# yahoo/CaffeOnSpark

Hardware: AMD Instinct MI355X
Metric: images/sec (higher is better)
Workload: dtype bf16; 1 GPU; model=alexnet(bvlc_reference/CaffeNet), global_batch=256, parallelism=dp1

## Files before the change

caffeonspark_amd/ops/csrc/ext.cpp:

```cpp

#include <torch/extension.h>
#include <ATen/hip/HIPContext.h>

#include <cstdint>

typedef struct ihipStream_t* hipStream_t;

namespace cosamd {

void gemm_bf16(const void* A, const void* B, void* C, const float* bias,
               int M, int N, int K, int lda, int ldb, int ldc,
               bool trans_a, bool trans_b, int store_mode, int splitk,
               bool relu, float alpha, int m_alloc, int n_alloc,
               hipStream_t stream);
void gemm_f32(const float* A, const float* B, float* C, const float* bias,
              int M, int N, int K, int64_t lda, int64_t ldb, int64_t ldc,
              bool trans_a, bool trans_b, int splitk, bool relu,
              hipStream_t stream);
void im2col_f32(const float* x, float* col, int N, int H, int W, int P,
                int Q, int R, int S, int sh, int sw, int ph, int pw, int dh,
                int dw, int c0, int Cg, int64_t sN, int64_t sC, int64_t sH,
                int64_t sW, hipStream_t stream);
void col2im_f32(const float* dcol, float* dx, int N, int H, int W, int P,
                int Q, int R, int S, int sh, int sw, int ph, int pw, int dh,
                int dw, int c0, int Cg, int64_t sN, int64_t sC, int64_t sH,
                int64_t sW, hipStream_t stream);
void gemm_conv_fwd(const void* X, const void* B, void* C,
                   const float* bias, const void* zpage, int M, int N,
                   int K, int ldb, int ldc, bool relu, bool accum,
                   const int* geom, hipStream_t stream);
void gemm_conv_dw(const void* A, const void* X, float* C,
                  const void* zpage, int M, int N, int K, int lda, int ldc,
                  int store_mode, int splitk, float alpha, float* db,
                  const int* geom, hipStream_t stream);
void gemm_conv_fwd_sc(const void* X, const void* B, void* C,
                      const float* bias, int M, int N, int K, int ldb,
                      int ldc, bool relu, const int* geom,
                      hipStream_t stream);
void gemm_conv_dw_sc(const void* A, const void* X, float* C, int M,
                     int N, int K, int lda, int ldc, int store_mode,
                     int splitk, float alpha, float* db, const int* geom,
                     hipStream_t stream);
void repack_weights(const int64_t* table, int ndesc, int64_t max_total,
                    hipStream_t stream);
void dw_unpack_acc(const float* dwp, float* arena, int Kout, int Cg,
                   int R, int S, int Kpad, bool accumulate,
                   hipStream_t stream);
void s2d_pack(const void* x, void* out, int N, int H, int W, int C, int st,
              int ph, int pw, int Hp, int Wp, int64_t sN, int64_t sC,
              int64_t sH, int64_t sW, hipStream_t stream);
void s2d_pack_weight(const void* src, void* dst, int Kout, int Cg, int R,
                     int S, int st, int Kpad, hipStream_t stream);
void d2s_pack_weight(const void* src, void* dst, int Ci, int Co, int R,
// ... 234 lines not shown
                     (int)x.size(0), (int)x.size(2), (int)x.size(3), (int)P,
                     (int)Q, (int)R, (int)S, (int)sh, (int)sw, (int)ph,
                     (int)pw, (int)dh, (int)dw, (int)c0, (int)Cg,
                     x.stride(0), x.stride(1), x.stride(2), x.stride(3),
                     cur_stream());
}

void py_col2im_f32(Tensor dcol, Tensor dx, int64_t P, int64_t Q, int64_t R,
                   int64_t S, int64_t sh, int64_t sw, int64_t ph, int64_t pw,
                   int64_t dh, int64_t dw, int64_t c0, int64_t Cg) {
  check_conv_f32(dx, dcol, P, Q, R, S, sh, sw, ph, pw, dh, dw, c0, Cg);
  cosamd::col2im_f32(dcol.data_ptr<float>(), dx.data_ptr<float>(),
                     (int)dx.size(0), (int)dx.size(2), (int)dx.size(3),
                     (int)P, (int)Q, (int)R, (int)S, (int)sh, (int)sw,
                     (int)ph, (int)pw, (int)dh, (int)dw, (int)c0, (int)Cg,
                     dx.stride(0), dx.stride(1), dx.stride(2), dx.stride(3),
                     cur_stream());
}

void py_gemm_conv_fwd(Tensor X, Tensor B, Tensor C,
                      c10::optional<Tensor> bias, Tensor zpage,
                      int64_t M, int64_t N, int64_t K, int64_t ldb,
                      int64_t ldc, bool relu, bool accum,
                      std::vector<int64_t> geom) {
  CHECK_CUDA(X); CHECK_BF16(X); CHECK_BF16(B); CHECK_BF16(C);
  const float* bptr = nullptr;
  if (bias.has_value()) {
    CHECK_F32(bias.value());
    bptr = bias.value().data_ptr<float>();
  }
  int g[14];
  TORCH_CHECK(geom.size() == 14, "geom must have 14 ints");
  for (int i = 0; i < 14; ++i) g[i] = (int)geom[i];
  cosamd::gemm_conv_fwd(X.data_ptr(), B.data_ptr(), C.data_ptr(), bptr,
                        zpage.data_ptr(), (int)M, (int)N, (int)K,
                        (int)ldb, (int)ldc, relu, accum, g,
                        cur_stream());
}

void py_gemm_conv_dw(Tensor A, Tensor X, Tensor C,
                     c10::optional<Tensor> db, Tensor zpage, int64_t M,
                     int64_t N,
                     int64_t K, int64_t lda, int64_t ldc,
                     int64_t store_mode, int64_t splitk, double alpha,
                     std::vector<int64_t> geom) {
  CHECK_CUDA(A); CHECK_BF16(A); CHECK_BF16(X); CHECK_F32(C);
  CHECK_CUDA(zpage); CHECK_BF16(zpage);
  TORCH_CHECK(zpage.numel() >= 8, "zpage must hold 16 zero bytes");
  float* dbp = nullptr;
  if (db.has_value()) {
    CHECK_F32(db.value());
    dbp = db.value().data_ptr<float>();
  }
  int g[14];
  TORCH_CHECK(geom.size() == 14, "geom must have 14 ints");
  for (int i = 0; i < 14; ++i) g[i] = (int)geom[i];
  cosamd::gemm_conv_dw(A.data_ptr(), X.data_ptr(), C.data_ptr<float>(),
                       zpage.data_ptr(), (int)M, (int)N, (int)K, (int)lda, (int)ldc,
                       (int)store_mode, (int)splitk, (float)alpha, dbp,
                       g, cur_stream());
// ... 548 lines not shown
  cosamd::softmax_loss_fwd(x.data_ptr(), label.data_ptr<float>(),
                           prob.data_ptr<float>(),
                           rowloss.data_ptr<float>(), loss.data_ptr<float>(),
                           count.data_ptr<int>(), x.size(0), x.size(1),
                           (int)ignore, has_ignore, cur_stream());
}

void py_softmax_loss_bwd(Tensor prob, Tensor label, Tensor dx, double scale,
                         int64_t ignore, bool has_ignore) {
  cosamd::softmax_loss_bwd(prob.data_ptr<float>(), label.data_ptr<float>(),
                           dx.data_ptr(), scale, prob.size(0), prob.size(1),
                           (int)ignore, has_ignore, cur_stream());
}

}

PYBIND11_MODULE(TORCH_EXTENSION_NAME, m) {
  m.def("gemm", &py_gemm);
  m.def("gemm_f32", &py_gemm_f32);
  m.def("im2col_f32", &py_im2col_f32);
  m.def("col2im_f32", &py_col2im_f32);
  m.def("relu_colsum_bwd", &py_relu_colsum_bwd);
  m.def("relu_db_dense", &py_relu_db_dense);
  m.def("gemm_conv_fwd", &py_gemm_conv_fwd);
  m.def("gemm_conv_dw", &py_gemm_conv_dw);
  m.def("gemm_conv_fwd_sc", &py_gemm_conv_fwd_sc);
  m.def("gemm_conv_dw_sc", &py_gemm_conv_dw_sc);
  m.def("im2col", &py_im2col);
  m.def("bn_stats", [](Tensor x, Tensor sum, Tensor sq, int64_t rows,
                       int64_t C) {
    cosamd::bn_stats(x.data_ptr(), sum.data_ptr<float>(),
                     sq.data_ptr<float>(), rows, C, cur_stream());
  });
  m.def("bn_bwd_sums", [](Tensor dy, Tensor xhat, Tensor s1, Tensor s2,
                          int64_t rows, int64_t C) {
    cosamd::bn_bwd_sums(dy.data_ptr(), xhat.data_ptr(),
                        s1.data_ptr<float>(), s2.data_ptr<float>(), rows,
                        C, cur_stream());
  });
  m.def("bn_norm", [](Tensor x, Tensor y, Tensor mean, Tensor invstd,
                      int64_t rows, int64_t C) {
    cosamd::bn_norm(x.data_ptr(), y.data_ptr(), mean.data_ptr<float>(),
                    invstd.data_ptr<float>(), rows, C, cur_stream());
  });
  m.def("bn_bwd", [](Tensor xhat, Tensor dy, Tensor dx, Tensor invstd,
                     Tensor s1, Tensor s2, double inv_m, int64_t rows,
                     int64_t C) {
// ... 75 lines not shown
```

caffeonspark_amd/ops/csrc/gemm.hip:

```cpp

#include "common.h"

#include <type_traits>

namespace cosamd {

typedef __bf16 bf16x8 __attribute__((ext_vector_type(8)));
typedef unsigned short short8v __attribute__((ext_vector_type(8)));
typedef float f32x4 __attribute__((ext_vector_type(4)));

constexpr int BM = 128, BN = 128, BK = 32;
constexpr int NTHREADS = 256;

__device__ __forceinline__ int swz_chunk(int row, int chunk) {
  return chunk ^ ((row >> 1) & 3);
}


struct Tile { int bm, bn, tile_m, tile_n; };

template <int TBN>
__device__ __forceinline__ Tile decode_tile(int M, int N) {
  int mblocks = (M + BM - 1) / BM;
  int nblocks = (N + TBN - 1) / TBN;
  int bid = xcd_swizzle(blockIdx.x, mblocks * nblocks);
  Tile t;
  t.bm = bid / nblocks;
  t.bn = bid % nblocks;
  t.tile_m = t.bm * BM;
  t.tile_n = t.bn * TBN;
  return t;
}

constexpr int mrows_of(int waves) { return BM / (waves / 2); }
constexpr int mfrags_of(int waves) { return mrows_of(waves) / 16; }

template <int MF, int MROWS, bool PRIO>
__device__ __forceinline__ void load_frags_mfma(
    const bf16* As, const bf16* Bs, int wm, int wn, int lane,
    f32x4 (&acc)[MF][4]) {
  int lrow = lane & 15, lchunk = lane >> 4;
  bf16x8 afrag[MF], bfrag[4];
#pragma unroll
  for (int f = 0; f < 4; ++f) {
    int rb = wn * 64 + f * 16 + lrow;
    bfrag[f] = *reinterpret_cast<const bf16x8*>(
        Bs + rb * BK + (swz_chunk(rb, lchunk) << 3));
  }
#pragma unroll
  for (int f = 0; f < MF; ++f) {
    int ra = wm * MROWS + f * 16 + lrow;
    afrag[f] = *reinterpret_cast<const bf16x8*>(
        As + ra * BK + (swz_chunk(ra, lchunk) << 3));
  }
  if (PRIO) __builtin_amdgcn_s_setprio(1);
#pragma unroll
  for (int fm = 0; fm < MF; ++fm)
#pragma unroll
    for (int fn = 0; fn < 4; ++fn)
      acc[fm][fn] = __builtin_amdgcn_mfma_f32_16x16x32_bf16(
          afrag[fm], bfrag[fn], acc[fm][fn], 0, 0, 0);
  if (PRIO) __builtin_amdgcn_s_setprio(0);
}

template <int MF, int MROWS, class Accum>
__device__ __forceinline__ void epilogue_bf16(
    const f32x4 (&acc)[MF][4], bf16* C, const float* bias, int M, int N,
    int ldc, int tile_m, int tile_n, int wm, int wn, int lane, int relu,
    float alpha, Accum accum) {
  int crow0 = tile_m + wm * MROWS + ((lane >> 4) << 2);
  int ccol0 = tile_n + wn * 64 + (lane & 15);
#pragma unroll
  for (int fm = 0; fm < MF; ++fm) {
#pragma unroll
    for (int fn = 0; fn < 4; ++fn) {
      int col = ccol0 + fn * 16;
      if (col >= N) continue;
      float badd = (bias != nullptr) ? bias[col] : 0.f;
#pragma unroll
      for (int r = 0; r < 4; ++r) {
        int row = crow0 + fm * 16 + r;
        if (row >= M) continue;
        float v = acc[fm][fn][r] * alpha + badd;
        if (relu && v < 0.f) v = 0.f;
        int64_t off = (int64_t)row * ldc + col;
        if (accum) v += bf2f(C[off]);
        C[off] = f2bf(v);
      }
    }
  }
}

template <int STORE, bool BIAS, int MF, int MROWS>
__device__ __forceinline__ void epilogue_f32(
    const f32x4 (&acc)[MF][4], float* C, const float* bias, int M, int N,
    int ldc, int tile_m, int tile_n, int wm, int wn, int lane, int relu,
    float alpha) {
  int crow0 = tile_m + wm * MROWS + ((lane >> 4) << 2);
  int ccol0 = tile_n + wn * 64 + (lane & 15);
#pragma unroll
  for (int fm = 0; fm < MF; ++fm) {
#pragma unroll
    for (int fn = 0; fn < 4; ++fn) {
      int col = ccol0 + fn * 16;
      if (col >= N) continue;
      float badd = (BIAS && bias != nullptr) ? bias[col] : 0.f;
#pragma unroll
      for (int r = 0; r < 4; ++r) {
        int row = crow0 + fm * 16 + r;
        if (row >= M) continue;
        float v = acc[fm][fn][r] * alpha;
        if (BIAS) {
// ... 64 lines not shown
    int m0 = (slot >> 4) * 8;
    unsigned short va[8], vb[8];
#pragma unroll
    for (int h = 0; h < 2; ++h) {
      unsigned short* v = h ? vb : va;
      int gk = k0 + kp * 2 + h;
      int gr = row0 + m0;
      if (gk < kend && gr + 8 <= rows && ((ld | gr) % 8 == 0)) {
        *reinterpret_cast<short8v*>(v) =
            *reinterpret_cast<const short8v*>(g + (int64_t)gk * ld + gr);
      } else if (gk < kend) {
#pragma unroll
        for (int j = 0; j < 8; ++j)
          v[j] = (gr + j < rows) ? g[(int64_t)gk * ld + gr + j] : 0;
      } else {
#pragma unroll
        for (int j = 0; j < 8; ++j) v[j] = 0;
      }
    }
    write_kpairs(lds, m0, kp, va, vb);
  }
}

template <int WAVES = 4>
__device__ __forceinline__ void stage_direct_fast(
    bf16* lds, const bf16* g, int row0, int ld, int k0, int tid) {
  int wave = tid >> 6, lane = tid & 63;
  constexpr int CPW = 8 / WAVES;
#pragma unroll
  for (int it = 0; it < CPW; ++it) {
    int chunk = wave * CPW + it;
    int idx = chunk * 512 + lane * 8;
    int row = idx >> 5;
    int kk = swz_chunk(row, (idx & 31) >> 3) << 3;
    auto* gp = (const __attribute__((address_space(1))) unsigned int*)(
        g + (int64_t)(row0 + row) * ld + k0 + kk);
    auto* lp = (__attribute__((address_space(3))) unsigned int*)(
        lds + chunk * 512);
    __builtin_amdgcn_global_load_lds(gp, lp, 16, 0, 0);
  }
}


struct CGeom {
  int H, W, C;
  int Q, PQ;
  int sh, sw, ph, pw, dil, S;
  int c0, Cg;
  int Kcol;
  unsigned long long mPQ, mQ, mCg, mS;
};

__device__ __forceinline__ unsigned mdiv(unsigned n,
                                         unsigned long long m) {
  return (unsigned)(((unsigned long long)n * m) >> 40);
}

static inline unsigned long long magic40(unsigned d) {
  return ((1ull << 40) + d - 1) / d;
}

__device__ __forceinline__ void decode_rows(int* rinfo, const CGeom& gm,
                                            int tile_m, int M, int rows,
                                            int tid) {
  for (int i = tid; i < rows; i += blockDim.x) {
    int m = tile_m + i;
    if (m >= M) m = M - 1;
    unsigned n = mdiv(m, gm.mPQ);
    unsigned pq = m - n * gm.PQ;
    unsigned p = mdiv(pq, gm.mQ);
    unsigned q = pq - p * gm.Q;
    rinfo[i * 3] = (int)(n * gm.H * gm.W);
    rinfo[i * 3 + 1] = (int)p * gm.sh - gm.ph;
    rinfo[i * 3 + 2] = (int)q * gm.sw - gm.pw;
  }
}

template <int WAVES>
__device__ __forceinline__ void stage_implicit_fast(
    bf16* lds_, const bf16* X, const bf16* zpage, const CGeom& gm,
    const int* rinfo, int k0, int tid) {
  auto* lds = reinterpret_cast<unsigned short*>(lds_);
  int wave = tid >> 6, lane = tid & 63;
  constexpr int CPW = 8 / WAVES;
#pragma unroll
  for (int it = 0; it < CPW; ++it) {
    int chunk = wave * CPW + it;
    int idx = chunk * 512 + lane * 8;
    int row = idx >> 5;
    int kk = swz_chunk(row, (idx & 31) >> 3) << 3;
    int k = k0 + kk;
    unsigned rs = mdiv(k, gm.mCg);
    int c = k - rs * gm.Cg;
    unsigned r = mdiv(rs, gm.mS);
    int s = rs - r * gm.S;
    int h = rinfo[row * 3 + 1] + (int)r * gm.dil;
    int w = rinfo[row * 3 + 2] + s * gm.dil;
    bool ok = (k < gm.Kcol) && (h >= 0) && (h < gm.H) && (w >= 0) &&
              (w < gm.W);
    int64_t off = ((int64_t)rinfo[row * 3] +
                   (int64_t)(h * gm.W + w)) * gm.C + gm.c0 + c;
    const bf16* src = ok ? X + off : zpage;
    auto* lp = (__attribute__((address_space(3))) unsigned int*)(
        lds + chunk * 512);
    auto* gp = (const __attribute__((address_space(1))) unsigned int*)src;
    __builtin_amdgcn_global_load_lds(gp, lp, 16, 0, 0);
  }
// ... 220 lines not shown
                             BM);
    bstage.stage(Bs, tile_n, N, k0, k_end, tid);
    __syncthreads();
    if (do_db && tid < BM && tile_m + tid < M) {
      float acc_b = 0.f;
      const bf16* row = As + tid * BK;
#pragma unroll
      for (int kk = 0; kk < BK; ++kk)
        acc_b += bf2f(row[(swz_chunk(tid, kk >> 3) << 3) | (kk & 7)]);
      atomicAdd(db + tile_m + tid, acc_b);
    }
    load_frags_mfma<4, 64, false>(As, Bs, wm, wn, lane, acc);
    __syncthreads();
  }

  epilogue_f32<STORE, false, 4, 64>(acc, C, nullptr, M, N, ldc, tile_m,
                                    tile_n, wm, wn, lane, 0, alpha);
}


struct ADirect {
  const bf16* A;
  int row0, ld;
  template <int WAVES>
  __device__ __forceinline__ void stage(bf16* lds, int k0, int tid) const {
    stage_direct_fast<WAVES>(lds, A, row0, ld, k0, tid);
  }
};

struct AImplicit {
  const bf16* X;
  const bf16* zpage;
  const CGeom& gm;
  const int* rinfo;
  template <int WAVES>
  __device__ __forceinline__ void stage(bf16* lds, int k0, int tid) const {
    stage_implicit_fast<WAVES>(lds, X, zpage, gm, rinfo, k0, tid);
  }
};

template <int N>
__device__ __forceinline__ void wait_vmcnt() {
  asm volatile("s_waitcnt vmcnt(%0)" ::"n"(N) : "memory");
}

template <int WAVES, int DEPTH, class AStage>
__device__ __forceinline__ void pipelined_loop(
    bf16 (*Asb)[BM * BK], bf16 (*Bsb)[BN * BK], const AStage& astage,
    const bf16* B, int tile_n, int ldb, int k_begin, int k_end, int tid,
    int wm, int wn, int lane, f32x4 (&acc)[mfrags_of(WAVES)][4]) {
  constexpr int PF = DEPTH / 2;
  constexpr int VMCNT = PF * 2 * (8 / WAVES);
#pragma unroll
  for (int p = 0; p < PF; ++p)
    if (p == 0 || k_begin + p * BK < k_end) {
      astage.template stage<WAVES>(Asb[p], k_begin + p * BK, tid);
      stage_direct_fast<WAVES>(Bsb[p], B, tile_n, ldb, k_begin + p * BK,
                               tid);
    }
  int cur = 0;
  for (int k0 = k_begin; k0 < k_end; k0 += BK) {
    if (k0 + PF * BK < k_end) {
      int nxt = (cur + PF) & (DEPTH - 1);
      astage.template stage<WAVES>(Asb[nxt], k0 + PF * BK, tid);
      stage_direct_fast<WAVES>(Bsb[nxt], B, tile_n, ldb, k0 + PF * BK,
                               tid);
    }
    wait_vmcnt<VMCNT>();
    __builtin_amdgcn_sched_barrier(0);
    __builtin_amdgcn_s_barrier();
    load_frags_mfma<mfrags_of(WAVES), mrows_of(WAVES), true>(
        Asb[cur], Bsb[cur], wm, wn, lane, acc);
    if (DEPTH == 2) __builtin_amdgcn_s_barrier();
    cur = (cur + 1) & (DEPTH - 1);
  }
}


template <bool TRANS_A, bool TRANS_B, int STORE_MODE, int WAVES = 4>
__global__ __launch_bounds__(WAVES * 64, 2) void gemm_kernel(
    const bf16* __restrict__ A, const bf16* __restrict__ B,
    void* __restrict__ C, const float* __restrict__ bias,
    int M, int N, int K, int lda, int ldb, int ldc,
    int ksplit, int relu, float alpha, int m_alloc, int n_alloc,
    int64_t sA, int64_t sB, int64_t sC) {
  A += (int64_t)blockIdx.z * sA;
  B += (int64_t)blockIdx.z * sB;
  C = (void*)((char*)C + (int64_t)blockIdx.z * sC);
  __shared__ bf16 Asb[2][BM * BK];
  __shared__ bf16 Bsb[2][BN * BK];

  Tile t = decode_tile<BN>(M, N);
  int tile_m = t.tile_m, tile_n = t.tile_n;
  int k_begin = blockIdx.y * ksplit;
  int k_end = min(K, k_begin + ksplit);

  constexpr int NT = WAVES * 64;
  constexpr int MROWS = mrows_of(WAVES), MF = mfrags_of(WAVES);
  int tid = threadIdx.x;
  int wave = tid >> 6, lane = tid & 63;
  int wm = wave >> 1, wn = wave & 1;

  f32x4 acc[MF][4] = {};

  bool a_fast = !TRANS_A && (tile_m + BM <= m_alloc) && (lda % 8 == 0) &&
                ((k_end - k_begin) % BK == 0) && (k_begin % 8 == 0);
  bool b_fast = !TRANS_B && (tile_n + BN <= n_alloc) && (ldb % 8 == 0) &&
                ((k_end - k_begin) % BK == 0) && (k_begin % 8 == 0);

  if (a_fast && b_fast && (k_end - k_begin) >= 2 * BK) {
    pipelined_loop<WAVES, 2>(Asb, Bsb, ADirect{A, tile_m, lda}, B, tile_n,
                             ldb, k_begin, k_end, tid, wm, wn, lane, acc);
  } else {
    bf16* As = Asb[0];
    bf16* Bs = Bsb[0];
    for (int k0 = k_begin; k0 < k_end; k0 += BK) {
      if (a_fast) {
        stage_direct_fast<WAVES>(As, A, tile_m, lda, k0, tid);
      } else if (TRANS_A) {
        stage_trans_pair_guarded(As, A, tile_m, M, lda, k0, k_end, tid,
                                 NT);
      } else {
        stage_direct_guarded(As, A, tile_m, M, lda, k0, k_end, tid, NT);
      }
      if (b_fast) {
        stage_direct_fast<WAVES>(Bs, B, tile_n, ldb, k0, tid);
      } else if (TRANS_B) {
        stage_trans_pair_guarded(Bs, B, tile_n, N, ldb, k0, k_end, tid,
                                 NT);
      } else {
        stage_direct_guarded(Bs, B, tile_n, N, ldb, k0, k_end, tid, NT);
      }
      __syncthreads();
      load_frags_mfma<MF, MROWS, false>(As, Bs, wm, wn, lane, acc);
      __syncthreads();
    }
  }

  if (STORE_MODE == 0 || STORE_MODE == 3)
    epilogue_bf16<MF, MROWS>(acc, reinterpret_cast<bf16*>(C), bias, M, N,
                             ldc, tile_m, tile_n, wm, wn, lane, relu, alpha,
                             std::bool_constant<STORE_MODE == 3>{});
  else
    epilogue_f32<STORE_MODE, true, MF, MROWS>(
        acc, reinterpret_cast<float*>(C), bias, M, N, ldc, tile_m, tile_n,
        wm, wn, lane, relu, alpha);
}


template <int WAVES, int DEPTH>
__global__ __launch_bounds__(WAVES * 64, 2) void gemm_conv_fwd_kernel(
    const bf16* __restrict__ X, const bf16* __restrict__ B,
    bf16* __restrict__ C, const float* __restrict__ bias,
    const bf16* __restrict__ zpage,
    int M, int N, int K, int ldb, int ldc, int relu, int accum,
    CGeom gm) {
  __shared__ bf16 Asb[DEPTH][BM * BK];
  __shared__ bf16 Bsb[DEPTH][BN * BK];
  __shared__ int rinfo[BM * 3];

  Tile t = decode_tile<BN>(M, N);
  int tid = threadIdx.x;
  int wave = tid >> 6, lane = tid & 63;
  int wm = wave >> 1, wn = wave & 1;

  decode_rows(rinfo, gm, t.tile_m, M, BM, tid);
  __syncthreads();

  f32x4 acc[mfrags_of(WAVES)][4] = {};
  pipelined_loop<WAVES, DEPTH>(Asb, Bsb, AImplicit{X, zpage, gm, rinfo}, B,
                               t.tile_n, ldb, 0, K, tid, wm, wn, lane, acc);
  epilogue_bf16<mfrags_of(WAVES), mrows_of(WAVES)>(
      acc, C, bias, M, N, ldc, t.tile_m, t.tile_n, wm, wn, lane, relu, 1.f,
      accum != 0);
}

template <int WAVES>
__global__ __launch_bounds__(WAVES * 64, 2) void gemm_conv_fwd_sc_kernel(
    const bf16* __restrict__ X, const bf16* __restrict__ B,
    bf16* __restrict__ C, const float* __restrict__ bias,
    int M, int N, int K, int ldb, int ldc, int relu, CGeom gm) {
  __shared__ bf16 Asb[2][BM * BK];
  __shared__ bf16 Bsb[2][BN * BK];
  __shared__ int rinfo[BM * 3];

  Tile tl = decode_tile<BN>(M, N);
  constexpr int NT = WAVES * 64;
  constexpr int MROWS = mrows_of(WAVES), MF = mfrags_of(WAVES);
  int tid = threadIdx.x;
  int wave = tid >> 6, lane = tid & 63;
  int wm = wave >> 1, wn = wave & 1;

  decode_rows(rinfo, gm, tl.tile_m, M, BM, tid);
  __syncthreads();

  f32x4 acc[MF][4] = {};
  int T = K / BK;
// ... 266 lines not shown
  }
  else if (!trans_a && trans_b)  COS_GEMM_SM(false, true);
  else if (trans_a && !trans_b)  COS_GEMM_SM(true, false);
  else                           COS_GEMM_SM(true, true);
#undef COS_GEMM_SM
#undef COS_GEMM_CASE
#undef COS_GEMM_CASE8
}

static CGeom make_geom(const int* g) {
  CGeom gm;
  gm.H = g[0]; gm.W = g[1]; gm.C = g[2];
  gm.Q = g[4]; gm.PQ = g[3] * g[4];
  gm.sh = g[5]; gm.sw = g[6]; gm.ph = g[7]; gm.pw = g[8];
  gm.dil = g[9]; gm.S = g[10];
  gm.c0 = g[11]; gm.Cg = g[12]; gm.Kcol = g[13];
  gm.mPQ = magic40(gm.PQ);
  gm.mQ = magic40(gm.Q);
  gm.mCg = magic40(gm.Cg);
  gm.mS = magic40(gm.S);
  return gm;
}

void gemm_conv_fwd(const void* X, const void* B, void* C,
                   const float* bias, const void* zpage, int M, int N,
                   int K, int ldb, int ldc, bool relu, bool accum,
                   const int* geom, hipStream_t stream) {
  CGeom gm = make_geom(geom);
  int mblocks = (M + BM - 1) / BM, nblocks = (N + BN - 1) / BN;
  dim3 grid(mblocks * nblocks);
  bool w8 = use_w8(M, N);
  static const int quad = [] {
    const char* e = getenv("COS_CONVQ");
    if (!e) return 1152;
    int v = atoi(e);
    return v == 1 ? 1 << 30 : v;
  }();
#define COS_CONV_FWD(WAVES, DEPTH)                                          \
  gemm_conv_fwd_kernel<WAVES, DEPTH><<<grid, WAVES * 64, 0, stream>>>(      \
      (const bf16*)X, (const bf16*)B, (bf16*)C, bias, (const bf16*)zpage,   \
      M, N, K, ldb, ldc, relu ? 1 : 0, accum ? 1 : 0, gm)
  if (quad && w8 && K >= 4 * BK && K <= quad) COS_CONV_FWD(8, 4);
  else if (w8)                                COS_CONV_FWD(8, 2);
  else                                        COS_CONV_FWD(4, 2);
#undef COS_CONV_FWD
}

void gemm_conv_fwd_sc(const void* X, const void* B, void* C,
                      const float* bias, int M, int N, int K, int ldb,
                      int ldc, bool relu, const int* geom,
                      hipStream_t stream) {
  CGeom gm = make_geom(geom);
  int mblocks = (M + BM - 1) / BM, nblocks = (N + BN - 1) / BN;
  dim3 grid(mblocks * nblocks);
  if (use_w8(M, N))
    gemm_conv_fwd_sc_kernel<8><<<grid, dim3(512), 0, stream>>>(
        (const bf16*)X, (const bf16*)B, (bf16*)C, bias, M, N, K, ldb,
        ldc, relu ? 1 : 0, gm);
  else
    gemm_conv_fwd_sc_kernel<4><<<grid, dim3(256), 0, stream>>>(
        (const bf16*)X, (const bf16*)B, (bf16*)C, bias, M, N, K, ldb,
        ldc, relu ? 1 : 0, gm);
}

void gemm_conv_dw_sc(const void* A, const void* X, float* C, int M,
                     int N, int K, int lda, int ldc, int store_mode,
                     int splitk, float alpha, float* db, const int* geom,
                     hipStream_t stream) {
// ... 45 lines not shown
```

caffeonspark_amd/ops/gpu.py:

```python

from __future__ import annotations

import math
import os
import torch

from . import reference

_ext = None


def _pad8(k: int) -> int:
    return (k + 7) // 8 * 8


def _pad32(k: int) -> int:
    return (k + 31) // 32 * 32


def _kpad_dma(k: int) -> int:
    return max(64, _pad32(k))


def _cl(x: torch.Tensor) -> torch.Tensor:
# ... 272 lines not shown
            and G == 1 and C % 8 == 0 and Kout % 8 == 0 and out_into is None
            and int(os.environ.get("COS_WINOGRAD", "0"))):
        _wino_run(xl, w, b, y, N, P, Q, C, Kout, relu)
        if ctx is not None:
            ctx["col"] = None
            ctx["xl"] = xl
            ctx["is_1x1"] = False
            ctx["wino"] = True
            ctx["s2d"] = None
            ctx["shape"] = (N, C, H, W, P, Q, R, S, sh, sw, ph, pw, dil, G,
                            Cg, Kg, Kpad, Kcol)
            ctx["wr"] = None
            ctx["w"] = w
        return y
    is_1x1 = (R == S == 1 and sh == sw == 1 and ph == pw == 0 and
              dil == 1 and G == 1 and C % 8 == 0 and not implicit)
    if is_1x1:
        x2 = xl.permute(0, 2, 3, 1).reshape(NPQ, C)
        _gemm(x2, wr, y2, bias_f, NPQ, Kout, C, C, C, ldc_out,
              False, False, 0, 1, relu=relu, na=wrb.shape[0])
        col = None
    elif implicit:
        col = None
        for g in range(G):
            geom = [H, W, C, P, Q, sh, sw, ph, pw, dil, S, g * Cg, Cg,
                    Kcol]
            _ext.gemm_conv_fwd(
                xl, wrb[g * Kg:], y2[:, g * Kg:],
                bias_f[g * Kg:(g + 1) * Kg] if bias_f is not None
                else None, _zpage(x.device), NPQ, Kg, Kpad, Kpad,
                ldc_out, relu, False, geom)
    elif implicit_sc:
        col = None
        geom = [H, W, C, P, Q, sh, sw, ph, pw, dil, C, 0, S * C, Kcol]
        _ext.gemm_conv_fwd_sc(xl, wrb, y2, bias_f, NPQ, Kout, Kpad,
                              Kpad, ldc_out, relu, geom)
    else:
        col = torch.empty((G, NPQ, Kpad), dtype=torch.bfloat16,
                          device=x.device)
        for g in range(G):
            _ext.im2col(xl, col[g], N, H, W, C, P, Q, R, S, sh, sw, ph, pw,
                        dil, Kpad, g * Cg, Cg)
            _gemm(col[g], wr[g * Kg:(g + 1) * Kg], y2[:, g * Kg:],
                  bias_f[g * Kg:(g + 1) * Kg] if bias_f is not None else None,
                  NPQ, Kg, Kpad, Kpad, Kpad, ldc_out, False, False, 0, 1,
                  relu=relu, na=wrb.shape[0] - g * Kg)
    if ctx is not None:
        ctx["col"] = col
        ctx["xl"] = xl
        ctx["is_1x1"] = is_1x1
        ctx["implicit"] = implicit and not is_1x1
        ctx["implicit_sc"] = implicit_sc
        ctx["s2d"] = None
        ctx["shape"] = (N, C, H, W, P, Q, R, S, sh, sw, ph, pw, dil, G, Cg,
# ... 124 lines not shown
    wK, wC = (w.shape[0], w.shape[1])
    ur = _pad128(K)
    U = torch.empty((16, ur, C), dtype=torch.bfloat16, device=dev)
    if ur != K:
        U.view(16, -1)[:, K * C:].zero_()
    V = torch.empty((16, T, C), dtype=torch.bfloat16, device=dev)
    M = torch.empty((16, T, K), dtype=torch.bfloat16, device=dev)
    x2 = xl.permute(0, 2, 3, 1)
    y2 = y.permute(0, 2, 3, 1)
    bias_f = b.float().contiguous() if b is not None else None
    _ext.wino_conv(x2, w.float().contiguous(), bias_f, y2, U, V, M,
                   N, P, Q, C, K, wK, wC, ur, flip, relu)


def _conv_dx(dyl, dyg, ld_dy, shape, wr, wrT, wrF, dx, dx_acc=False):
    (N, C, H, W, P, Q, R, S, sh, sw, ph, pw, dil, G, Cg, Kg, Kpad,
     Kcol) = shape
    NPQ = N * P * Q
    k2 = R * S * Kg
    cgp = _pad128(Cg)
    if wrF is not None and wrF.shape == (G * cgp, _kpad_dma(k2)) \
            and N * H * W < (1 << 20):
        dx2 = dx.permute(0, 2, 3, 1).reshape(N * H * W, C)
        for g in range(G):
            geom = [P, Q, ld_dy, H, W, 1, 1,
                    dil * (R - 1) - ph, dil * (S - 1) - pw, dil, S,
                    g * Kg, Kg, k2]
            _ext.gemm_conv_fwd(dyl, wrF[g * cgp:], dx2[:, g * Cg:],
                               None, _zpage(dyl.device), N * H * W,
                               Cg, _kpad_dma(k2), _kpad_dma(k2), C, False,
                               dx_acc, geom)
        return
    dcol = torch.empty((NPQ, Kpad), dtype=torch.bfloat16,
                       device=dyl.device)
    for g in range(G):
        wT = wrT
        if wT is None:
            wT = _transpose(wr[g * Kg:(g + 1) * Kg].contiguous())
        _gemm(dyg(g), wT, dcol, None,
              NPQ, Kpad, Kg, ld_dy, Kg, Kpad, False, False, 0, 1,
              ma=NPQ, na=_pad128(Kpad))
        _ext.col2im(dcol, dx, N, H, W, C, P, Q, R, S, sh, sw, ph, pw,
                    dil, Kpad, g * Cg, Cg)


def conv2d_backward(x, w, dy, stride, pad, dilation, groups,
                    need_dx=True, need_dw=True, bias=True, ctx=None,
                    dw_out=None, db_out=None, dx_into=None):
    _check_bf16(dy, "conv dy")
    if ctx is None or "col" not in ctx:
        ctx = ctx if ctx is not None else {}
        conv2d_forward(_cl(x), w, None, stride, pad, dilation, groups,
                       ctx=ctx)
    (N, C, H, W, P, Q, R, S, sh, sw, ph, pw, dil, G, Cg, Kg, Kpad,
# ... 1186 lines not shown
```

Baseline: 74830 images/sec.

## Generalize implicit conv forward kernel: variable tiles, grouped grid, vectorized epilogue

Parameterizes the implicit-GEMM conv forward kernel over tile shape (TBM/TBN, wave layout, pipeline depth) and adds a planner that picks a narrower N tile (96/64/48) when it reduces padding waste. Groups are launched in one kernel via a second grid dimension instead of a Python loop per group, and a vectorized epilogue stages accumulators through LDS to write 16-byte bf16 stores. The pipelined loop's tail is restructured so the last iterations wait on the exact number of outstanding loads. This adds many template instantiations and larger LDS use, and could hurt occupancy or pick worse tiles for some layers.

```diff
diff --git a/caffeonspark_amd/ops/csrc/ext.cpp b/caffeonspark_amd/ops/csrc/ext.cpp
--- a/caffeonspark_amd/ops/csrc/ext.cpp
+++ b/caffeonspark_amd/ops/csrc/ext.cpp
@@ -28,7 +28,12 @@
 void gemm_conv_fwd(const void* X, const void* B, void* C,
                    const float* bias, const void* zpage, int M, int N,
                    int K, int ldb, int ldc, bool relu, bool accum,
-                   const int* geom, hipStream_t stream);
+                   const int* geom, int groups, int gs_c, int gs_b,
+                   int gs_n, int cfg, int vec, hipStream_t stream);
+struct ConvCfg { int id, bm, bn, waves, depth; };
+ConvCfg conv_fwd_plan(int M, int N, int K);
+int conv_fwd_num_cfgs();
+ConvCfg conv_fwd_cfg(int id);
 void gemm_conv_dw(const void* A, const void* X, float* C,
                   const void* zpage, int M, int N, int K, int lda, int ldc,
                   int store_mode, int splitk, float alpha, float* db,
@@ -309,8 +314,11 @@
                       c10::optional<Tensor> bias, Tensor zpage,
                       int64_t M, int64_t N, int64_t K, int64_t ldb,
                       int64_t ldc, bool relu, bool accum,
-                      std::vector<int64_t> geom) {
+                      std::vector<int64_t> geom, int64_t groups,
+                      int64_t gs_c, int64_t gs_b, int64_t gs_n,
+                      int64_t cfg, int64_t vec) {
   CHECK_CUDA(X); CHECK_BF16(X); CHECK_BF16(B); CHECK_BF16(C);
+  TORCH_CHECK(groups >= 1, "groups must be positive");
   const float* bptr = nullptr;
   if (bias.has_value()) {
     CHECK_F32(bias.value());
@@ -321,8 +329,23 @@
   for (int i = 0; i < 14; ++i) g[i] = (int)geom[i];
   cosamd::gemm_conv_fwd(X.data_ptr(), B.data_ptr(), C.data_ptr(), bptr,
                         zpage.data_ptr(), (int)M, (int)N, (int)K,
-                        (int)ldb, (int)ldc, relu, accum, g,
+                        (int)ldb, (int)ldc, relu, accum, g, (int)groups,
+                        (int)gs_c, (int)gs_b, (int)gs_n, (int)cfg, (int)vec,
                         cur_stream());
+}
+
+std::vector<int64_t> py_conv_fwd_plan(int64_t M, int64_t N, int64_t K) {
+  cosamd::ConvCfg p = cosamd::conv_fwd_plan((int)M, (int)N, (int)K);
+  return {p.bm, p.bn, p.waves, p.depth};
+}
+
+std::vector<std::vector<int64_t>> py_conv_fwd_cfgs() {
+  std::vector<std::vector<int64_t>> out;
+  for (int i = 0; i < cosamd::conv_fwd_num_cfgs(); ++i) {
+    cosamd::ConvCfg p = cosamd::conv_fwd_cfg(i);
+    out.push_back({p.bm, p.bn, p.waves, p.depth});
+  }
+  return out;
 }
 
 void py_gemm_conv_dw(Tensor A, Tensor X, Tensor C,
@@ -917,7 +940,14 @@
   m.def("col2im_f32", &py_col2im_f32);
   m.def("relu_colsum_bwd", &py_relu_colsum_bwd);
   m.def("relu_db_dense", &py_relu_db_dense);
-  m.def("gemm_conv_fwd", &py_gemm_conv_fwd);
+  m.def("gemm_conv_fwd", &py_gemm_conv_fwd, py::arg("X"), py::arg("B"),
+        py::arg("C"), py::arg("bias"), py::arg("zpage"), py::arg("M"),
+        py::arg("N"), py::arg("K"), py::arg("ldb"), py::arg("ldc"),
+        py::arg("relu"), py::arg("accum"), py::arg("geom"),
+        py::arg("groups") = 1, py::arg("gs_c") = 0, py::arg("gs_b") = 0,
+        py::arg("gs_n") = 0, py::arg("cfg") = -1, py::arg("vec") = -1);
+  m.def("conv_fwd_plan", &py_conv_fwd_plan);
+  m.def("conv_fwd_cfgs", &py_conv_fwd_cfgs);
   m.def("gemm_conv_dw", &py_gemm_conv_dw);
   m.def("gemm_conv_fwd_sc", &py_gemm_conv_fwd_sc);
   m.def("gemm_conv_dw_sc", &py_gemm_conv_dw_sc);
diff --git a/caffeonspark_amd/ops/csrc/gemm.hip b/caffeonspark_amd/ops/csrc/gemm.hip
--- a/caffeonspark_amd/ops/csrc/gemm.hip
+++ b/caffeonspark_amd/ops/csrc/gemm.hip
@@ -19,15 +19,15 @@
 
 struct Tile { int bm, bn, tile_m, tile_n; };
 
-template <int TBN>
+template <int TBN, int TBM = BM>
 __device__ __forceinline__ Tile decode_tile(int M, int N) {
-  int mblocks = (M + BM - 1) / BM;
+  int mblocks = (M + TBM - 1) / TBM;
   int nblocks = (N + TBN - 1) / TBN;
   int bid = xcd_swizzle(blockIdx.x, mblocks * nblocks);
   Tile t;
   t.bm = bid / nblocks;
   t.bn = bid % nblocks;
-  t.tile_m = t.bm * BM;
+  t.tile_m = t.bm * TBM;
   t.tile_n = t.bn * TBN;
   return t;
 }
@@ -35,15 +35,32 @@
 constexpr int mrows_of(int waves) { return BM / (waves / 2); }
 constexpr int mfrags_of(int waves) { return mrows_of(waves) / 16; }
 
-template <int MF, int MROWS, bool PRIO>
+template <int TBM_, int TBN_, int WM_, int WN_>
+struct TileCfg {
+  static constexpr int TBM = TBM_, TBN = TBN_, WM = WM_, WN = WN_;
+  static constexpr int WAVES = WM * WN;
+  static constexpr int MROWS = TBM / WM, NCOLS = TBN / WN;
+  static constexpr int MF = MROWS / 16, NF = NCOLS / 16;
+  static constexpr int A_CHUNKS = TBM / 16, B_CHUNKS = TBN / 16;
+  static constexpr int A_CPW = A_CHUNKS / WAVES;
+  static constexpr int B_CPW = (B_CHUNKS + WAVES - 1) / WAVES;
+  static constexpr int A_ELEMS = TBM * BK;
+  static constexpr int B_ELEMS = B_CPW * WAVES * 512;
+  static_assert(MROWS % 16 == 0 && NCOLS % 16 == 0, "whole fragments");
+  static_assert(A_CHUNKS % WAVES == 0, "A chunks divide over the waves");
+};
+template <int WAVES>
+using Tile128 = TileCfg<BM, BN, WAVES / 2, 2>;
+
+template <int MF, int MROWS, bool PRIO, int NF = 4, int NCOLS = 64>
 __device__ __forceinline__ void load_frags_mfma(
     const bf16* As, const bf16* Bs, int wm, int wn, int lane,
-    f32x4 (&acc)[MF][4]) {
+    f32x4 (&acc)[MF][NF]) {
   int lrow = lane & 15, lchunk = lane >> 4;
-  bf16x8 afrag[MF], bfrag[4];
-#pragma unroll
-  for (int f = 0; f < 4; ++f) {
-    int rb = wn * 64 + f * 16 + lrow;
+  bf16x8 afrag[MF], bfrag[NF];
+#pragma unroll
+  for (int f = 0; f < NF; ++f) {
+    int rb = wn * NCOLS + f * 16 + lrow;
     bfrag[f] = *reinterpret_cast<const bf16x8*>(
         Bs + rb * BK + (swz_chunk(rb, lchunk) << 3));
   }
@@ -57,23 +74,23 @@
 #pragma unroll
   for (int fm = 0; fm < MF; ++fm)
 #pragma unroll
-    for (int fn = 0; fn < 4; ++fn)
+    for (int fn = 0; fn < NF; ++fn)
       acc[fm][fn] = __builtin_amdgcn_mfma_f32_16x16x32_bf16(
           afrag[fm], bfrag[fn], acc[fm][fn], 0, 0, 0);
   if (PRIO) __builtin_amdgcn_s_setprio(0);
 }
 
-template <int MF, int MROWS, class Accum>
+template <int MF, int MROWS, int NF = 4, int NCOLS = 64, class Accum>
 __device__ __forceinline__ void epilogue_bf16(
-    const f32x4 (&acc)[MF][4], bf16* C, const float* bias, int M, int N,
+    const f32x4 (&acc)[MF][NF], bf16* C, const float* bias, int M, int N,
     int ldc, int tile_m, int tile_n, int wm, int wn, int lane, int relu,
     float alpha, Accum accum) {
   int crow0 = tile_m + wm * MROWS + ((lane >> 4) << 2);
-  int ccol0 = tile_n + wn * 64 + (lane & 15);
+  int ccol0 = tile_n + wn * NCOLS + (lane & 15);
 #pragma unroll
   for (int fm = 0; fm < MF; ++fm) {
 #pragma unroll
-    for (int fn = 0; fn < 4; ++fn) {
+    for (int fn = 0; fn < NF; ++fn) {
       int col = ccol0 + fn * 16;
       if (col >= N) continue;
       float badd = (bias != nullptr) ? bias[col] : 0.f;
@@ -88,6 +105,68 @@
         C[off] = f2bf(v);
       }
     }
+  }
+}
+
+template <class Cfg>
+constexpr int vec_slab_floats() { return Cfg::WAVES * 16 * (Cfg::NCOLS + 4); }
+
+template <class Cfg>
+__device__ __forceinline__ void epilogue_bf16_vec(
+    const f32x4 (&acc)[Cfg::MF][Cfg::NF], float* lds, bf16* C,
+    const float* bias, int M, int N, int ldc, int tile_m, int tile_n, int wm,
+    int wn, int wave, int lane, int relu, int accum) {
+  constexpr int LD = Cfg::NCOLS + 4;
+  constexpr int GPR = Cfg::NCOLS / 8;
+  constexpr int TASKS = 16 * GPR;
+  float* slab = lds + wave * 16 * LD;
+  int wr = (lane >> 4) << 2, wc = lane & 15;
+#pragma unroll
+  for (int fm = 0; fm < Cfg::MF; ++fm) {
+#pragma unroll
+    for (int fn = 0; fn < Cfg::NF; ++fn)
+#pragma unroll
+      for (int r = 0; r < 4; ++r)
+        slab[(wr + r) * LD + fn * 16 + wc] = acc[fm][fn][r];
+    __builtin_amdgcn_wave_barrier();
+#pragma unroll
+    for (int t0 = 0; t0 < TASKS; t0 += 64) {
+      int t = t0 + lane;
+      int row = t / GPR, cg = t - row * GPR;
+      int grow = tile_m + wm * Cfg::MROWS + fm * 16 + row;
+      int col = tile_n + wn * Cfg::NCOLS + cg * 8;
+      if ((TASKS % 64 == 0 || t < TASKS) && grow < M && col < N) {
+        f32x4 lo = *reinterpret_cast<const f32x4*>(slab + row * LD + cg * 8);
+        f32x4 hi =
+            *reinterpret_cast<const f32x4*>(slab + row * LD + cg * 8 + 4);
+        float v[8] = {lo[0], lo[1], lo[2], lo[3], hi[0], hi[1], hi[2], hi[3]};
+        if (bias != nullptr) {
+          f32x4 b0 = *reinterpret_cast<const f32x4*>(bias + col);
+          f32x4 b1 = *reinterpret_cast<const f32x4*>(bias + col + 4);
+#pragma unroll
+          for (int j = 0; j < 4; ++j) { v[j] += b0[j]; v[4 + j] += b1[j]; }
+        }
+        if (relu) {
+#pragma unroll
+          for (int j = 0; j < 8; ++j) v[j] = v[j] < 0.f ? 0.f : v[j];
+        }
+        short8v* dst =
+            reinterpret_cast<short8v*>(C + (int64_t)grow * ldc + col);
+        bf16 o[8];
+        if (accum) {
+          short8v old = *dst;
+          __builtin_memcpy(o, &old, 16);
+#pragma unroll
+          for (int j = 0; j < 8; ++j) v[j] += bf2f(o[j]);
+        }
+#pragma unroll
+        for (int j = 0; j < 8; ++j) o[j] = f2bf(v[j]);
+        short8v out;
+        __builtin_memcpy(&out, o, 16);
+        *dst = out;
+      }
+    }
+    __builtin_amdgcn_wave_barrier();
   }
 }
 
@@ -198,19 +277,22 @@
   }
 }
 
-template <int WAVES = 4>
+template <int WAVES = 4, int CHUNKS = 8>
 __device__ __forceinline__ void stage_direct_fast(
-    bf16* lds, const bf16* g, int row0, int ld, int k0, int tid) {
+    bf16* lds, const bf16* g, int row0, int ld, int k0, int tid,
+    const bf16* zpage = nullptr, int rows = 0) {
   int wave = tid >> 6, lane = tid & 63;
-  constexpr int CPW = 8 / WAVES;
+  constexpr int CPW = (CHUNKS + WAVES - 1) / WAVES;
 #pragma unroll
   for (int it = 0; it < CPW; ++it) {
     int chunk = wave * CPW + it;
     int idx = chunk * 512 + lane * 8;
     int row = idx >> 5;
     int kk = swz_chunk(row, (idx & 31) >> 3) << 3;
-    auto* gp = (const __attribute__((address_space(1))) unsigned int*)(
-        g + (int64_t)(row0 + row) * ld + k0 + kk);
+    const bf16* src = g + (int64_t)(row0 + row) * ld + k0 + kk;
+    if (zpage != nullptr && (chunk >= CHUNKS || row0 + row >= rows))
+      src = zpage;
+    auto* gp = (const __attribute__((address_space(1))) unsigned int*)src;
     auto* lp = (__attribute__((address_space(3))) unsigned int*)(
         lds + chunk * 512);
     __builtin_amdgcn_global_load_lds(gp, lp, 16, 0, 0);
@@ -252,13 +334,13 @@
   }
 }
 
-template <int WAVES>
+template <int WAVES, int CHUNKS = 8>
 __device__ __forceinline__ void stage_implicit_fast(
     bf16* lds_, const bf16* X, const bf16* zpage, const CGeom& gm,
     const int* rinfo, int k0, int tid) {
   auto* lds = reinterpret_cast<unsigned short*>(lds_);
   int wave = tid >> 6, lane = tid & 63;
-  constexpr int CPW = 8 / WAVES;
+  constexpr int CPW = CHUNKS / WAVES;
 #pragma unroll
   for (int it = 0; it < CPW; ++it) {
     int chunk = wave * CPW + it;
@@ -525,9 +607,9 @@
 struct ADirect {
   const bf16* A;
   int row0, ld;
-  template <int WAVES>
+  template <int WAVES, int CHUNKS>
   __device__ __forceinline__ void stage(bf16* lds, int k0, int tid) const {
-    stage_direct_fast<WAVES>(lds, A, row0, ld, k0, tid);
+    stage_direct_fast<WAVES, CHUNKS>(lds, A, row0, ld, k0, tid);
   }
 };
 
@@ -536,9 +618,9 @@
   const bf16* zpage;
   const CGeom& gm;
   const int* rinfo;
-  template <int WAVES>
+  template <int WAVES, int CHUNKS>
   __device__ __forceinline__ void stage(bf16* lds, int k0, int tid) const {
-    stage_implicit_fast<WAVES>(lds, X, zpage, gm, rinfo, k0, tid);
+    stage_implicit_fast<WAVES, CHUNKS>(lds, X, zpage, gm, rinfo, k0, tid);
   }
 };
 
@@ -547,36 +629,53 @@
   asm volatile("s_waitcnt vmcnt(%0)" ::"n"(N) : "memory");
 }
 
-template <int WAVES, int DEPTH, class AStage>
+template <class Cfg, int DEPTH, class AStage>
 __device__ __forceinline__ void pipelined_loop(
-    bf16 (*Asb)[BM * BK], bf16 (*Bsb)[BN * BK], const AStage& astage,
-    const bf16* B, int tile_n, int ldb, int k_begin, int k_end, int tid,
-    int wm, int wn, int lane, f32x4 (&acc)[mfrags_of(WAVES)][4]) {
+    bf16* Asb, bf16* Bsb, const AStage& astage, const bf16* B,
+    const bf16* zpage, int b_rows, int tile_n, int ldb, int k_begin,
+    int k_end, int tid, int wm, int wn, int lane,
+    f32x4 (&acc)[Cfg::MF][Cfg::NF]) {
+  constexpr int WAVES = Cfg::WAVES;
   constexpr int PF = DEPTH / 2;
-  constexpr int VMCNT = PF * 2 * (8 / WAVES);
+  constexpr int VMCNT = PF * (Cfg::A_CPW + Cfg::B_CPW);
 #pragma unroll
   for (int p = 0; p < PF; ++p)
     if (p == 0 || k_begin + p * BK < k_end) {
-      astage.template stage<WAVES>(Asb[p], k_begin + p * BK, tid);
-      stage_direct_fast<WAVES>(Bsb[p], B, tile_n, ldb, k_begin + p * BK,
-                               tid);
+      astage.template stage<WAVES, Cfg::A_CHUNKS>(
+          Asb + p * Cfg::A_ELEMS, k_begin + p * BK, tid);
+      stage_direct_fast<WAVES, Cfg::B_CHUNKS>(
+          Bsb + p * Cfg::B_ELEMS, B, tile_n, ldb, k_begin + p * BK, tid,
+          zpage, b_rows);
     }
   int cur = 0;
-  for (int k0 = k_begin; k0 < k_end; k0 += BK) {
-    if (k0 + PF * BK < k_end) {
-      int nxt = (cur + PF) & (DEPTH - 1);
-      astage.template stage<WAVES>(Asb[nxt], k0 + PF * BK, tid);
-      stage_direct_fast<WAVES>(Bsb[nxt], B, tile_n, ldb, k0 + PF * BK,
-                               tid);
-    }
-    wait_vmcnt<VMCNT>();
+  auto compute = [&](int slot) {
     __builtin_amdgcn_sched_barrier(0);
     __builtin_amdgcn_s_barrier();
-    load_frags_mfma<mfrags_of(WAVES), mrows_of(WAVES), true>(
-        Asb[cur], Bsb[cur], wm, wn, lane, acc);
+    load_frags_mfma<Cfg::MF, Cfg::MROWS, true, Cfg::NF, Cfg::NCOLS>(
+        Asb + slot * Cfg::A_ELEMS, Bsb + slot * Cfg::B_ELEMS, wm, wn, lane,
+        acc);
+  };
+  int k0 = k_begin;
+  for (; k0 + PF * BK < k_end; k0 += BK) {
+    int nxt = (cur + PF) & (DEPTH - 1);
+    astage.template stage<WAVES, Cfg::A_CHUNKS>(
+        Asb + nxt * Cfg::A_ELEMS, k0 + PF * BK, tid);
+    stage_direct_fast<WAVES, Cfg::B_CHUNKS>(
+        Bsb + nxt * Cfg::B_ELEMS, B, tile_n, ldb, k0 + PF * BK, tid, zpage,
+        b_rows);
+    wait_vmcnt<VMCNT>();
+    compute(cur);
     if (DEPTH == 2) __builtin_amdgcn_s_barrier();
     cur = (cur + 1) & (DEPTH - 1);
   }
+  static_assert(PF == 1 || PF == 2, "tail waits written out for PF <= 2");
+  if (PF == 2) {
+    wait_vmcnt<VMCNT / 2>();
+    compute(cur);
+    cur = (cur + 1) & (DEPTH - 1);
+  }
+  wait_vmcnt<0>();
+  compute(cur);
 }
 
 
@@ -612,8 +711,9 @@
                 ((k_end - k_begin) % BK == 0) && (k_begin % 8 == 0);
 
   if (a_fast && b_fast && (k_end - k_begin) >= 2 * BK) {
-    pipelined_loop<WAVES, 2>(Asb, Bsb, ADirect{A, tile_m, lda}, B, tile_n,
-                             ldb, k_begin, k_end, tid, wm, wn, lane, acc);
+    pipelined_loop<Tile128<WAVES>, 2>(
+        &Asb[0][0], &Bsb[0][0], ADirect{A, tile_m, lda}, B, nullptr, 0,
+        tile_n, ldb, k_begin, k_end, tid, wm, wn, lane, acc);
   } else {
     bf16* As = Asb[0];
     bf16* Bs = Bsb[0];
@@ -651,31 +751,51 @@
 }
 
 
-template <int WAVES, int DEPTH>
-__global__ __launch_bounds__(WAVES * 64, 2) void gemm_conv_fwd_kernel(
+template <class Cfg, int DEPTH>
+__global__ __launch_bounds__(Cfg::WAVES * 64, 2) void gemm_conv_fwd_kernel(
     const bf16* __restrict__ X, const bf16* __restrict__ B,
     bf16* __restrict__ C, const float* __restrict__ bias,
     const bf16* __restrict__ zpage,
     int M, int N, int K, int ldb, int ldc, int relu, int accum,
-    CGeom gm) {
-  __shared__ bf16 Asb[DEPTH][BM * BK];
-  __shared__ bf16 Bsb[DEPTH][BN * BK];
-  __shared__ int rinfo[BM * 3];
-
-  Tile t = decode_tile<BN>(M, N);
+    CGeom gm, int gs_c, int gs_b, int gs_n, int vec) {
+  int b_rows = (N + 127) / 128 * 128;
+  constexpr int RING = DEPTH * (Cfg::A_ELEMS + Cfg::B_ELEMS);
+  constexpr int STAGING = RING + Cfg::TBM * 3 * (sizeof(int) / sizeof(bf16));
+  constexpr int SLABS = vec_slab_floats<Cfg>() * (sizeof(float) / sizeof(bf16));
+  __shared__ __attribute__((aligned(16)))
+  bf16 smem[STAGING > SLABS ? STAGING : SLABS];
+  bf16* Asb = smem;
+  bf16* Bsb = smem + DEPTH * Cfg::A_ELEMS;
+  int* rinfo = reinterpret_cast<int*>(smem + RING);
+
+  int g = blockIdx.y;
+  gm.c0 += g * gs_c;
+  B += (int64_t)g * gs_b * ldb;
+  C += g * gs_n;
+  if (bias != nullptr) bias += g * N;
+
+  Tile t = decode_tile<Cfg::TBN, Cfg::TBM>(M, N);
   int tid = threadIdx.x;
   int wave = tid >> 6, lane = tid & 63;
-  int wm = wave >> 1, wn = wave & 1;
-
-  decode_rows(rinfo, gm, t.tile_m, M, BM, tid);
+  int wm = wave / Cfg::WN, wn = wave % Cfg::WN;
+
+  decode_rows(rinfo, gm, t.tile_m, M, Cfg::TBM, tid);
   __syncthreads();
 
-  f32x4 acc[mfrags_of(WAVES)][4] = {};
-  pipelined_loop<WAVES, DEPTH>(Asb, Bsb, AImplicit{X, zpage, gm, rinfo}, B,
-                               t.tile_n, ldb, 0, K, tid, wm, wn, lane, acc);
-  epilogue_bf16<mfrags_of(WAVES), mrows_of(WAVES)>(
-      acc, C, bias, M, N, ldc, t.tile_m, t.tile_n, wm, wn, lane, relu, 1.f,
-      accum != 0);
+  f32x4 acc[Cfg::MF][Cfg::NF] = {};
+  pipelined_loop<Cfg, DEPTH>(Asb, Bsb, AImplicit{X, zpage, gm, rinfo}, B,
+                             zpage, b_rows, t.tile_n, ldb, 0, K, tid, wm,
+                             wn, lane, acc);
+  if (vec) {
+    __syncthreads();
+    epilogue_bf16_vec<Cfg>(acc, reinterpret_cast<float*>(smem), C, bias, M,
+                           N, ldc, t.tile_m, t.tile_n, wm, wn, wave, lane,
+                           relu, accum);
+  } else {
+    epilogue_bf16<Cfg::MF, Cfg::MROWS, Cfg::NF, Cfg::NCOLS>(
+        acc, C, bias, M, N, ldc, t.tile_m, t.tile_n, wm, wn, lane, relu,
+        1.f, accum != 0);
+  }
 }
 
 template <int WAVES>
@@ -988,28 +1108,108 @@
   return gm;
 }
 
-void gemm_conv_fwd(const void* X, const void* B, void* C,
-                   const float* bias, const void* zpage, int M, int N,
-                   int K, int ldb, int ldc, bool relu, bool accum,
-                   const int* geom, hipStream_t stream) {
-  CGeom gm = make_geom(geom);
-  int mblocks = (M + BM - 1) / BM, nblocks = (N + BN - 1) / BN;
-  dim3 grid(mblocks * nblocks);
-  bool w8 = use_w8(M, N);
+#ifdef COS_CONV_SWEEP
+#define COS_CONV_SWEEP_CFGS(CFG_)                                           \
+  CFG_(12, 128, 96, 4, 2, 4)  CFG_(13, 256, 96, 4, 2, 2)                    \
+  CFG_(14, 256, 64, 4, 1, 2)  CFG_(15, 256, 48, 4, 1, 2)                    \
+  CFG_(16, 128, 96, 2, 2, 4)  CFG_(17, 128, 64, 2, 2, 4)
+#else
+#define COS_CONV_SWEEP_CFGS(CFG_)
+#endif
+#define COS_CONV_CFGS(CFG_)                                                 \
+  CFG_(0, 128, 128, 4, 2, 4)  CFG_(1, 128, 128, 4, 2, 2)                    \
+  CFG_(2, 128, 128, 2, 2, 2)  CFG_(3, 128, 96, 2, 2, 2)                     \
+  CFG_(4, 128, 96, 4, 2, 2)   CFG_(5, 128, 64, 2, 2, 2)                     \
+  CFG_(6, 128, 64, 4, 2, 2)   CFG_(7, 128, 64, 4, 2, 4)                     \
+  CFG_(8, 256, 64, 4, 2, 2)   CFG_(9, 128, 48, 4, 1, 2)                     \
+  CFG_(10, 128, 48, 4, 1, 4)  CFG_(11, 256, 48, 8, 1, 2)                    \
+  COS_CONV_SWEEP_CFGS(CFG_)
+
+struct ConvCfg { int id, bm, bn, waves, depth; };
+
+static const ConvCfg kConvCfgs[] = {
+#define CFG_(ID, TBM, TBN, WM, WN, DEPTH) {ID, TBM, TBN, WM * WN, DEPTH},
+    COS_CONV_CFGS(CFG_)
+#undef CFG_
+};
+constexpr int kNumConvCfgs = sizeof(kConvCfgs) / sizeof(kConvCfgs[0]);
+
+static bool conv_vec(int id) {
+  (void)id;
+  return true;
+}
+
+int conv_fwd_num_cfgs() { return kNumConvCfgs; }
+ConvCfg conv_fwd_cfg(int id) {
+  if (id < 0 || id >= kNumConvCfgs)
+    throw std::runtime_error("conv_fwd_cfg: no such configuration");
+  return kConvCfgs[id];
+}
+
+static int conv_bn(int N) {
+  const char* e = getenv("COS_CONV_BN");
+  int forced = e ? atoi(e) : 0;
+  if (forced != 0 && forced != 48 && forced != 64 && forced != 96 &&
+      forced != 128)
+    throw std::runtime_error("COS_CONV_BN must be 0, 48, 64, 96 or 128");
+  if (forced) return forced;
+  int best = 128, best_pad = (N + 127) / 128 * 128;
+  for (int bn : {96, 64, 48}) {
+    int pad = (N + bn - 1) / bn * bn;
+    if (pad < best_pad) { best = bn; best_pad = pad; }
+  }
+  return best;
+}
+
+ConvCfg conv_fwd_plan(int M, int N, int K) {
   static const int quad = [] {
     const char* e = getenv("COS_CONVQ");
     if (!e) return 1152;
     int v = atoi(e);
     return v == 1 ? 1 << 30 : v;
   }();
-#define COS_CONV_FWD(WAVES, DEPTH)                                          \
-  gemm_conv_fwd_kernel<WAVES, DEPTH><<<grid, WAVES * 64, 0, stream>>>(      \
-      (const bf16*)X, (const bf16*)B, (bf16*)C, bias, (const bf16*)zpage,   \
-      M, N, K, ldb, ldc, relu ? 1 : 0, accum ? 1 : 0, gm)
-  if (quad && w8 && K >= 4 * BK && K <= quad) COS_CONV_FWD(8, 4);
-  else if (w8)                                COS_CONV_FWD(8, 2);
-  else                                        COS_CONV_FWD(4, 2);
-#undef COS_CONV_FWD
+  bool w8 = use_w8(M, N);
+  bool q = quad && K >= 4 * BK && K <= quad;
+  bool big_m = M >= 8192;
+  int id;
+  switch (conv_bn(N)) {
+    case 96: id = w8 ? 4 : 3; break;
+    case 64: id = big_m ? 8 : w8 ? (q ? 7 : 6) : 5; break;
+    case 48: id = big_m ? 11 : q ? 10 : 9; break;
+    default: id = w8 ? (q ? 0 : 1) : 2; break;
+  }
+  return kConvCfgs[id];
+}
+
+void gemm_conv_fwd(const void* X, const void* B, void* C,
+                   const float* bias, const void* zpage, int M, int N,
+                   int K, int ldb, int ldc, bool relu, bool accum,
+                   const int* geom, int groups, int gs_c, int gs_b,
+                   int gs_n, int cfg, int vec, hipStream_t stream) {
+  CGeom gm = make_geom(geom);
+  if (K % BK != 0 || K < 2 * BK)
+    throw std::runtime_error("gemm_conv_fwd: K must be whole 32-wide tiles, "
+                             "at least two");
+  if (cfg >= kNumConvCfgs)
+    throw std::runtime_error("gemm_conv_fwd: no such configuration");
+  ConvCfg p = cfg >= 0 ? kConvCfgs[cfg] : conv_fwd_plan(M, N, K);
+  int mblocks = (M + p.bm - 1) / p.bm, nblocks = (N + p.bn - 1) / p.bn;
+  dim3 grid(mblocks * nblocks, max(1, groups));
+  bool vec_ok = ((N | ldc | (groups > 1 ? gs_n : 0)) % 8 == 0) &&
+                (((uintptr_t)C | (uintptr_t)bias) % 16 == 0);
+  int use_vec = vec_ok && (vec < 0 ? conv_vec(p.id) : vec != 0);
+  switch (p.id) {
+#define CFG_(ID, TBM, TBN, WM, WN, DEPTH)                                   \
+    case ID:                                                                \
+      gemm_conv_fwd_kernel<TileCfg<TBM, TBN, WM, WN>, DEPTH>                \
+          <<<grid, WM * WN * 64, 0, stream>>>(                              \
+              (const bf16*)X, (const bf16*)B, (bf16*)C, bias,               \
+              (const bf16*)zpage, M, N, K, ldb, ldc, relu ? 1 : 0,          \
+              accum ? 1 : 0, gm, gs_c, gs_b, gs_n, use_vec);                \
+      break;
+    COS_CONV_CFGS(CFG_)
+#undef CFG_
+  }
 }
 
 void gemm_conv_fwd_sc(const void* X, const void* B, void* C,
diff --git a/caffeonspark_amd/ops/gpu.py b/caffeonspark_amd/ops/gpu.py
--- a/caffeonspark_amd/ops/gpu.py
+++ b/caffeonspark_amd/ops/gpu.py
@@ -318,14 +318,10 @@
         col = None
     elif implicit:
         col = None
-        for g in range(G):
-            geom = [H, W, C, P, Q, sh, sw, ph, pw, dil, S, g * Cg, Cg,
-                    Kcol]
-            _ext.gemm_conv_fwd(
-                xl, wrb[g * Kg:], y2[:, g * Kg:],
-                bias_f[g * Kg:(g + 1) * Kg] if bias_f is not None
-                else None, _zpage(x.device), NPQ, Kg, Kpad, Kpad,
-                ldc_out, relu, False, geom)
+        geom = [H, W, C, P, Q, sh, sw, ph, pw, dil, S, 0, Cg, Kcol]
+        _ext.gemm_conv_fwd(xl, wrb, y2, bias_f, _zpage(x.device), NPQ, Kg,
+                           Kpad, Kpad, ldc_out, relu, False, geom, G, Cg,
+                           Kg, Kg)
     elif implicit_sc:
         col = None
         geom = [H, W, C, P, Q, sh, sw, ph, pw, dil, C, 0, S * C, Kcol]
@@ -496,14 +492,11 @@
     if wrF is not None and wrF.shape == (G * cgp, _kpad_dma(k2)) \
             and N * H * W < (1 << 20):
         dx2 = dx.permute(0, 2, 3, 1).reshape(N * H * W, C)
-        for g in range(G):
-            geom = [P, Q, ld_dy, H, W, 1, 1,
-                    dil * (R - 1) - ph, dil * (S - 1) - pw, dil, S,
-                    g * Kg, Kg, k2]
-            _ext.gemm_conv_fwd(dyl, wrF[g * cgp:], dx2[:, g * Cg:],
-                               None, _zpage(dyl.device), N * H * W,
-                               Cg, _kpad_dma(k2), _kpad_dma(k2), C, False,
-                               dx_acc, geom)
+        geom = [P, Q, ld_dy, H, W, 1, 1,
+                dil * (R - 1) - ph, dil * (S - 1) - pw, dil, S, 0, Kg, k2]
+        _ext.gemm_conv_fwd(dyl, wrF, dx2, None, _zpage(dyl.device),
+                           N * H * W, Cg, _kpad_dma(k2), _kpad_dma(k2), C,
+                           False, dx_acc, geom, G, Kg, cgp, Cg)
         return
     dcol = torch.empty((NPQ, Kpad), dtype=torch.bfloat16,
                        device=dyl.device)
```

Result: faster. 85910 images/sec (median of 6 runs) (+14.8%).
